# Farama-Foundation/Gymnasium-Robotics

Measured on AMD Instinct MI355X. Metric: env-steps/s (whole node), higher is better.
Workload: dtype f32

## Files before the change

gymnasium_robotics_amd/_native.py:

```python
import ctypes
import os

_HERE = os.path.dirname(os.path.abspath(__file__))
LIB_PATH = os.environ.get("GRX_HIP_LIB") or os.path.join(_HERE, "_lib", "libgrx_hip.so")
_lib = None


class OverflowLaneStruct(ctypes.Structure):
    _fields_ = [(n, ctypes.c_void_p) for n in ("skip", "entry_count", "entry_list", "list", "count", "next_flags", "next_count", "next_list", "ttl")] + [
        (n, ctypes.c_int) for n in ("soft_maxefc", "soft_jpool", "soft_maxcon", "ttl_init", "grid", "entry_cap", "next_cap")] + [
        (n, ctypes.c_void_p) for n in ("ready", "progress", "poll_list")] + [(n, ctypes.c_int) for n in ("ready_cap", "progress_total", "poll_grid", "pad_")]


class FetchBuffersStruct(ctypes.Structure):
    _fields_ = [(n, ctypes.c_void_p) for n in (
        "qpos", "qvel", "qacc_ws", "mocap", "aux", "goal", "action", "obs", "achieved", "reward", "success", "status", "mask", "order", "cost", "packed", "hullcache", "handoff")] + [
        ("handoff_stride", ctypes.c_int), ("handoff_large", ctypes.c_int), ("split_state", ctypes.c_void_p), ("split_parts", ctypes.c_int), ("sites_every_substep", ctypes.c_int), ("lane", OverflowLaneStruct)]


class FetchResetArgsStruct(ctypes.Structure):
    _fields_ = [(n, ctypes.c_void_p) for n in ("idx", "samples", "init_qpos", "init_qvel", "init_mocap")] + [("obj_qadr", ctypes.c_int), ("keep_outcome", ctypes.c_int), ("final_packed", ctypes.c_void_p)]


class PointTaskStruct(ctypes.Structure):
    _fields_ = [("n_substeps", ctypes.c_int), ("sparse_reward", ctypes.c_int), ("continuing_task", ctypes.c_int), ("agent", ctypes.c_int),
                ("goal_radius", ctypes.c_double), ("vel_clip", ctypes.c_float)]
# ... 227 lines not shown
```

gymnasium_robotics_amd/core.py:

```python
import numpy as np

from .spaces import Dict


class GoalVecEnv:

    metadata = {"render_modes": []}

    def __new__(cls, *args, **kwargs):
        obj = super().__new__(cls)
        obj._ezpickle_args, obj._ezpickle_kwargs = args, kwargs
        return obj

    def __getstate__(self):
        return {"_ezpickle_args": self._ezpickle_args, "_ezpickle_kwargs": self._ezpickle_kwargs}

    def __setstate__(self, d):
        out = type(self)(*d["_ezpickle_args"], **d["_ezpickle_kwargs"])
        self.__dict__.update(out.__dict__)
        out.__dict__.pop("_h", None)
        out.__dict__.pop("_h_big", None)
        if getattr(self, "lane", None) is not None and hasattr(self, "_lane_make_bufs"):
            self.lane._make_bufs = self._lane_make_bufs()

# ... 273 lines not shown
        import torch

        self.head = torch.zeros((n + 3) // 4 + 2, dtype=torch.int32, device=device)
        self.flags = self.head.view(torch.uint8)[:n]
        self.counts = self.head[-2:]
        self.next_list, self.entry_list = torch.zeros(n, dtype=torch.int32, device=device), torch.zeros(n, dtype=torch.int32, device=device)
        base = self.counts.data_ptr()
        self.next_count_ptr, self.entry_count_ptr = base, base + 4


ENTRY_CAP = 256


class OverflowLane:

    def __init__(self, n, device, model, make_bufs, ttl=LANE_TTL, mode="lane", lane_first=False, margin=LANE_MARGIN, poll_grid=LANE_POLL_GRID, handoff=False):
        import os
        self.mode = os.environ.get("GRX_LANE_MODE", mode)
        self.handoff = bool(handoff)
        self.entry_cap = max(ENTRY_CAP, n // 16) if self.handoff else ENTRY_CAP
        self.lane_first = bool(int(os.environ.get("GRX_LANE_FIRST", int(lane_first))))
        self.spacer = int(os.environ.get("GRX_LANE_SPACER", 0))

        import torch

        from . import _native
        from .mjcf.compiler import DIMS

        self.n, self.device = n, device
        self.cur, self.nxt, self.scratch = _LaneBuf(n, device), _LaneBuf(n, device), _LaneBuf(n, device)
        self.ttl = torch.zeros(n, dtype=torch.int8, device=device)
        dims = model.tables["dims"]
        req = lambda k, default: int(dims[DIMS.index(k + "_req")]) or default
        cap = (req("maxefc", 144), req("jpool", 2032), min(req("maxcon", 32), 32))
        margin, ttl = float(os.environ.get("GRX_LANE_MARGIN", margin)), int(os.environ.get("GRX_LANE_TTL", ttl))
        self.soft = tuple(int(margin * v) for v in cap) + (int(ttl),)
        self._make_bufs = make_bufs
        self.side = torch.cuda.Stream(device=device, priority=int(os.environ.get("GRX_LANE_PRIO", "-1")))
        self._Lane = _native.OverflowLaneStruct
        self._pin = [dict(buf=torch.zeros(2, dtype=torch.int32, pin_memory=True), event=None, age=0) for _ in range(4)]
        self._pin_next, self._seen, self._age = 0, 0, 0
        self.cap_cur = 64
        self.poll_grid = int(os.environ.get("GRX_LANE_POLL", poll_grid)) if self.mode == "lane" else 0
        self._poll = torch.zeros(self.poll_grid + 1, dtype=torch.int32, device=device) if self.poll_grid > 0 else None
        self._fast_grid = (n + 7) & ~7
# ... 97 lines not shown
            pass
        elif slot["event"] is None or slot["event"].query():
            done = torch.cuda.Event()
            done.record(main)
            self.side.wait_event(done)
            with torch.cuda.stream(self.side):
                slot["buf"].copy_(nxt.counts, non_blocking=True)
                slot["event"] = torch.cuda.Event()
                slot["event"].record(self.side)
            self._age += 1
            slot["age"] = self._age
        self.cur, self.nxt, self.cap_cur = nxt, cur, next_cap

    def rerun_only(self, mask, fast_bufs, launch_fast, launch_large):
        sc = self.scratch
        sc.head.zero_()
        fast_bufs.lane = self._fast(None, sc, 0, join=False)
        launch_fast(fast_bufs)
        fast_bufs.lane = self._Lane()
        b = self._make_bufs(mask)
        b.lane = self._large(sc.entry_list, sc.entry_count_ptr, sc, ENTRY_CAP, 0)
        launch_large(b)

    def get_state(self):
        cur = self.cur
        return dict(head=cur.head.clone(), next_list=cur.next_list.clone(), entry_list=cur.entry_list.clone(), ttl=self.ttl.clone(), cap_cur=int(self.cap_cur), seen=int(self._seen))

    def set_state(self, st):
        import torch

        cur = self.cur
        cur.head.copy_(st["head"]); cur.next_list.copy_(st["next_list"]); cur.entry_list.copy_(st["entry_list"]); self.ttl.copy_(st["ttl"])
        self.cap_cur, self._seen = int(st["cap_cur"]), int(st["seen"])
        for slot in self._pin:
            if slot["event"] is not None:
                slot["event"].synchronize()
# ... 11 lines not shown
```

gymnasium_robotics_amd/csrc/grx_engine.h:

```cpp
#pragma once
#include <math.h>
#include <stdint.h>

#if defined(GRX_EMU)
#define GRX_ON_DEVICE 0
#else
#define GRX_ON_DEVICE 1
#endif
#if GRX_ON_DEVICE && defined(GRX_PROFILE)
#define GRX_DEVICE_PROFILE 1
#else
#define GRX_DEVICE_PROFILE 0
#endif
#if defined(GRX_HULL_HINTS)
#define GRX_DEVICE_HULL_HINTS GRX_ON_DEVICE
#define GRX_TWIN_HULL_HINTS (!GRX_ON_DEVICE)
#else
#define GRX_DEVICE_HULL_HINTS 0
#define GRX_TWIN_HULL_HINTS 0
#endif
#if defined(GRX_EMU) && defined(GRX_EMU_TRACE)
#define GRX_TWIN_TRACE 1
#else
#define GRX_TWIN_TRACE 0
// ... 121 lines not shown
#define GRX_CELL_MAX 64
GRX_HD int grx_hull_cell(float x, float y, float z) {
  const float ax = fabsf(x), ay = fabsf(y), az = fabsf(z);
  int face; float ma, u, v;
  if (ax >= ay && ax >= az) { face = x < 0.0f ? 1 : 0; ma = ax; u = y; v = z; }
  else if (ay >= az) { face = y < 0.0f ? 3 : 2; ma = ay; u = x; v = z; }
  else { face = z < 0.0f ? 5 : 4; ma = az; u = x; v = y; }
  const float s = (0.5f * GRX_CELL_G) / fmaxf(ma, 1e-30f);
  int iu = (int)floorf(u * s + 0.5f * GRX_CELL_G), iv = (int)floorf(v * s + 0.5f * GRX_CELL_G);
  iu = iu < 0 ? 0 : (iu > GRX_CELL_G - 1 ? GRX_CELL_G - 1 : iu); iv = iv < 0 ? 0 : (iv > GRX_CELL_G - 1 ? GRX_CELL_G - 1 : iv);
  return (face * GRX_CELL_G + iu) * GRX_CELL_G + iv;
}
#define GRX_HULLCACHE_WORDS 90

struct GrxLane { const unsigned char* skip; int* entry_count; int* entry_list; const int* list; const int* count; unsigned char* next_flags; int* next_count; int* next_list; signed char* ttl; int soft_maxefc, soft_jpool, soft_maxcon, ttl_init, grid, entry_cap, next_cap;
                 int* ready; int* progress; const int* poll_list; int ready_cap, progress_total, poll_grid, pad_; };

struct GrxCtx {
  float *qpos, *qvel, *qacc_ws, *mocap_pos, *mocap_quat, *ctrl;
  float *ploc, *qloc, *janchor, *jaxis;
  float *xpos, *xquat, *xmat, *cinert, *crb, *cvel, *cacc, *cfrc;
  float *gxpos, *gxmat, *sxpos, *sxmat;
  float *cdof, *cdof_dot;
  float *M, *A;
  float *qfrc_bias, *qfrc_passive, *qfrc_actuator, *qfrc_smooth, *qacc_smooth, *qfrc_constraint, *qacc, *Ma, *grad, *search,
      *Mv, *tmpv;
  float *con_dist, *con_pos, *con_frame;
  int *con_pair, *con_efc, *con_nr, *con_b1, *con_b2, *con_span, *con_ioff;
  float *Jp, *efc_pos, *efc_D, *efc_aref, *efc_jar, *efc_jv, *efc_force, *efc_floss;
  int *efc_kind, *efc_id, *efc_quad, *efc_row;
  float *rk_q0, *rk_v0, *rk_Fv, *rk_Fa;
// ... 480 lines not shown
```

gymnasium_robotics_amd/csrc/grx_env.hip:

```cpp
#include <hip/hip_runtime.h>

#include <sys/random.h>

#include <cstdio>
#include <cstdlib>
#include <cstring>
#include <map>
#include <string>
#include <vector>

#include "grx_capi.h"
#include "grx_env.h"
#include "grx_replay.h"
#include "grx_episodes.h"
#include "grx_norm.h"
#include "grx_copy.h"

namespace {

constexpr int kEntryCap = 256;
constexpr int kSplitParts = 4;
constexpr int kSplitWide = 12288;
constexpr double kLaneMargin = 0.8;
constexpr int kLaneTtl = 4;
// ... 194 lines not shown
  grx_model *h = nullptr, *hbig = nullptr;
  int nq = 0, nv = 0, nmocap = 0, nu = 0, obs_dim = 0, pdim = 0, obj_qadr = -1;
  double g0[3] = {0, 0, 0}, toff[3] = {0, 0, 0}, height_offset = 0, dt = 0;
  int soft[4] = {0, 0, 0, 0};
  std::vector<void*> allocs;
  float *qpos, *qvel, *qacc_ws, *mocap, *aux, *goal, *action, *obs, *achieved, *reward, *packed, *final_packed, *final_rows, *hullcache, *cost_ema = nullptr;
  unsigned char *success, *mask;
  int *status, *cost = nullptr, *order = nullptr;
  float* split_rows = nullptr;
  int* split_state = nullptr;
  uint64_t *rng, *rng_rows;
  float *init_qpos, *init_qvel, *init_mocap;
  int *idx_main, *idx_ahead;
  float *samp_main, *samp_ahead;
  int* lane_head;
  int *lane_next_list, *lane_entry_list;
  signed char* lane_ttl;
  size_t lane_head_bytes = 0;
  float *a_qpos, *a_qvel, *a_qacc_ws, *a_mocap, *a_aux, *a_goal, *a_obs, *a_achieved, *a_reward;
  unsigned char* a_success;
  int* a_status;
  grx_fetch_buffers bufs{}, bufs_masked{}, lane_plain{}, lane_masked{}, ahead_bufs{};
  bool balance = false, ahead = false;
  bool fused_tail = true;
  int slots_per_xcd = 0, split = 1;
  hipStream_t side = nullptr;
  hipEvent_t ev_before = nullptr, ev_ahead = nullptr;
  void* pin[kPinSlots] = {};
  hipEvent_t pin_ev[kPinSlots] = {};
  bool pin_live[kPinSlots] = {};
// ... 58 lines not shown
  explicit DeviceGuard(int dev) { if (hipGetDevice(&prev) != hipSuccess) prev = -1; if (prev != dev) (void)hipSetDevice(dev); }
  ~DeviceGuard() { int cur; if (prev >= 0 && hipGetDevice(&cur) == hipSuccess && cur != prev) (void)hipSetDevice(prev); }
};

grx_fetch_buffers make_bufs(grx_env* e, float* qpos, float* qvel, float* qacc, float* mocap, float* aux, float* goal, float* obs, float* ach, float* rew, unsigned char* succ,
                            int* status, const unsigned char* mask, const int* order, int* cost, float* packed, float* hullcache) {
  grx_fetch_buffers b;
  std::memset(&b, 0, sizeof b);
  b.qpos = qpos; b.qvel = qvel; b.qacc_ws = qacc; b.mocap = mocap; b.aux = aux; b.goal = goal; b.action = e->action; b.obs = obs; b.achieved = ach;
  b.reward = rew; b.success = succ; b.status = status; b.mask = mask; b.order = order; b.cost = cost; b.packed = packed; b.hullcache = hullcache;
  return b;
}

int launch_step(grx_env* e, bool masked, bool order_now, hipStream_t s) {
  grx_fetch_buffers& fb = masked ? e->bufs_masked : e->bufs;
  ENV_HIP(hipMemsetAsync(e->lane_head, 0, e->lane_head_bytes, s));
  int* counts = e->lane_head + (e->lane_head_bytes / 4 - 2);
  std::memset(&fb.lane, 0, sizeof fb.lane);
  fb.lane.entry_count = counts + 1; fb.lane.entry_list = e->lane_entry_list; fb.lane.entry_cap = kEntryCap;
  const int rc = grx_fetch_step(e->h, &e->d.task, &fb, e->n, s);
  std::memset(&fb.lane, 0, sizeof fb.lane);
  if (rc != 0) return fail(GRX_ENV_EHIP, std::string("grx_fetch_step: ") + grx_last_error());
  grx_fetch_buffers& b = masked ? e->lane_masked : e->lane_plain;
  std::memset(&b.lane, 0, sizeof b.lane);
  b.lane.grid = kEntryCap; b.lane.list = e->lane_entry_list; b.lane.count = counts + 1;
  b.lane.next_flags = (unsigned char*)e->lane_head; b.lane.next_count = counts; b.lane.next_list = e->lane_next_list; b.lane.ttl = e->lane_ttl; b.lane.next_cap = 0;
  b.lane.soft_maxefc = e->soft[0]; b.lane.soft_jpool = e->soft[1]; b.lane.soft_maxcon = e->soft[2]; b.lane.ttl_init = e->soft[3];
  ENV_GRX(grx_fetch_step(e->hbig, &e->d.task, &b, e->n, s));
  if (e->balance && order_now) ENV_GRX(grx_order_by_cost_slots(e->cost, e->cost_ema, kBalanceAlpha, e->n, e->slots_per_xcd, e->order, s));
  return 0;
}

int sample_resets(grx_env* e, const int* idx_dev, int k, float* samples, hipStream_t s) {
  const double* c = e->d.consts;
  ENV_GRX(grx_fetch_sample_resets_device(e->rng, idx_dev, k, (int)c[0], (int)c[2], c[7], c[8], e->toff, e->g0, e->height_offset, samples, s));
  return 0;
}

int reset_inline(grx_env* e, const int* idx_dev, int k, const float* samples, bool keep_outcome, hipStream_t s) {
  grx_fetch_reset_args a;
  std::memset(&a, 0, sizeof a);
  a.idx = idx_dev; a.samples = samples; a.init_qpos = e->init_qpos; a.init_qvel = e->init_qvel; a.init_mocap = e->init_mocap; a.obj_qadr = e->obj_qadr;
  a.keep_outcome = keep_outcome ? 1 : 0; a.final_packed = keep_outcome ? e->final_packed : nullptr;
// ... 45 lines not shown
}

int alloc_all(grx_env* e) {
  const int n = e->n;
  ENV_TRY(e->zalloc(&e->qpos, (size_t)n * e->nq)); ENV_TRY(e->zalloc(&e->qvel, (size_t)n * e->nv)); ENV_TRY(e->zalloc(&e->qacc_ws, (size_t)n * e->nv));
  ENV_TRY(e->zalloc(&e->mocap, (size_t)n * 7 * e->nmocap)); ENV_TRY(e->zalloc(&e->aux, (size_t)n * 8)); ENV_TRY(e->zalloc(&e->goal, (size_t)n * 3));
  ENV_TRY(e->zalloc(&e->action, (size_t)n * 4)); ENV_TRY(e->zalloc(&e->obs, (size_t)n * e->obs_dim)); ENV_TRY(e->zalloc(&e->achieved, (size_t)n * 3));
  ENV_TRY(e->zalloc(&e->reward, n)); ENV_TRY(e->zalloc(&e->success, n)); ENV_TRY(e->zalloc(&e->status, n)); ENV_TRY(e->zalloc(&e->mask, n));
  ENV_HIP(hipMemset(e->mask, 1, n));
  ENV_TRY(e->zalloc(&e->packed, (size_t)n * e->pdim)); ENV_TRY(e->zalloc(&e->final_packed, (size_t)n * e->pdim)); ENV_TRY(e->zalloc(&e->final_rows, (size_t)n * e->pdim));
  ENV_TRY(e->zalloc(&e->hullcache, (size_t)n * kHullWords));
  ENV_TRY(e->zalloc(&e->rng, (size_t)n * 4)); ENV_TRY(e->zalloc(&e->rng_rows, (size_t)n * 4));
  ENV_TRY(e->zalloc(&e->init_qpos, e->nq)); ENV_TRY(e->zalloc(&e->init_qvel, e->nv)); ENV_TRY(e->zalloc(&e->init_mocap, 7 * e->nmocap));
  ENV_TRY(e->zalloc(&e->idx_main, n)); ENV_TRY(e->zalloc(&e->idx_ahead, n)); ENV_TRY(e->zalloc(&e->samp_main, (size_t)n * 5)); ENV_TRY(e->zalloc(&e->samp_ahead, (size_t)n * 5));
  e->lane_head_bytes = (size_t)((n + 3) / 4 + 2) * 4;
  ENV_TRY(e->zalloc(&e->lane_head, e->lane_head_bytes / 4)); ENV_TRY(e->zalloc(&e->lane_next_list, n)); ENV_TRY(e->zalloc(&e->lane_entry_list, n)); ENV_TRY(e->zalloc(&e->lane_ttl, n));
  e->balance = n % 8 == 0 && n >= 1024 && n <= 65536 * 8;
  { const char* v = std::getenv("GRX_FETCH_FUSED_TAIL"); e->fused_tail = !(v && v[0] == '0' && v[1] == 0); }
  if (e->balance) {
    ENV_TRY(e->zalloc(&e->cost, n)); ENV_TRY(e->zalloc(&e->cost_ema, n)); ENV_TRY(e->zalloc(&e->order, n));
    const int lds = grx_model_lds_bytes(e->h);
    const int granules = (lds + 1279) / 1280;
    const int per_cu = granules > 0 ? (160 * 1024) / (granules * 1280) : 8;
    e->slots_per_xcd = 32 * (per_cu < 8 ? per_cu : 8);
    std::vector<int> ord(n);
    const int per = n / 8;
    for (int j = 0; j < n; ++j) ord[j] = (j % 8) * per + j / 8;
    ENV_HIP(hipMemcpy(e->order, ord.data(), (size_t)n * 4, hipMemcpyHostToDevice));
  }
  e->bufs = make_bufs(e, e->qpos, e->qvel, e->qacc_ws, e->mocap, e->aux, e->goal, e->obs, e->achieved, e->reward, e->success, e->status, nullptr, e->order, e->cost, e->packed, e->hullcache);
  e->bufs_masked = e->bufs;
// ... 438 lines not shown
```

gymnasium_robotics_amd/csrc/grx_kernels.hip:

```cpp
#if !defined(GRX_TU_FETCH) && !defined(GRX_TU_HAND) && !defined(GRX_TU_POINT) && !defined(GRX_TU_ADROIT) && !defined(GRX_TU_KITCHEN) && !defined(GRX_TU_SIM) && !defined(GRX_TU_API)
#define GRX_TU_FETCH 1
#define GRX_TU_HAND 1
#define GRX_TU_POINT 1
#define GRX_TU_ADROIT 1
#define GRX_TU_KITCHEN 1
#define GRX_TU_SIM 1
#define GRX_TU_API 1
#endif
#if GRX_TU_FETCH && !defined(GRX_NO_HULL_HINTS)
#define GRX_HULL_HINTS 1
#endif
#include <hip/hip_runtime.h>

#include <cmath>
#include <cstdio>
#include <cstring>
#include <string>

#include "../../include/grx_capi.h"
#include "grx_fetch_task.h"
#include "grx_point_task.h"
#include "grx_hand_task.h"
#include "grx_adroit_task.h"
#include "grx_kitchen_task.h"
// ... 213 lines not shown
}
template <class S>
__global__ void __launch_bounds__(64, GRX_FETCH_WAVES(S))
grx_fetch_step_kernel(int mslot, GrxFetchTask t, GrxFetchBuffers b, int n_worlds, int words) {
  extern __shared__ float lds[];
  const int lane_ = threadIdx.x;
  const int parts = b.split_parts > 1 ? b.split_parts : 1;
  const unsigned G = gridDim.x / (unsigned)parts, part = blockIdx.x / G, slot = blockIdx.x - part * G;
  grx_fetch_step_world<S, false>(mslot, t, b, grx_slot_world(b.order, slot, G), n_worlds, words, lds, lane_, (int)part, parts);
  grx_lane_progress(b.lane);
}
template <class S>
__global__ void __launch_bounds__(64, 2)
grx_fetch_lane_kernel(int mslot, GrxFetchTask t, GrxFetchBuffers b, int n_worlds, int words) {
  extern __shared__ float lds[];
  const int e = blockIdx.x, nstand = (int)gridDim.x - b.lane.poll_grid;
  if (e >= nstand) {
    const int ent = grx_lane_poll(b.lane, e - nstand);
    if (ent < 0) return;
    if ((ent >> 30) & 1) { if (threadIdx.x == 0) atomicExch(b.lane.ready + (e - nstand), 1); return; }
    grx_fetch_step_world<S, true>(mslot, t, b, ent & 0x3FFFFFFF, n_worlds, words, lds, (int)threadIdx.x);
    return;
  }
  if (e >= *b.lane.count || grx_lane_taken(b.lane, e)) return;
  grx_fetch_step_world<S, true>(mslot, t, b, b.lane.list[e] & 0x3FFFFFFF, n_worlds, words, lds, (int)threadIdx.x);
}

template <class S>
__global__ void __launch_bounds__(64, GRX_FETCH_WAVES(S))
grx_fetch_forward_kernel(int mslot, GrxFetchTask t, GrxFetchBuffers b, int n_worlds, int words, int nstep) {
// ... 328 lines not shown
template <class S>
__global__ void __launch_bounds__(64, 2)
grx_adroit_step_kernel(int mslot, GrxAdroitTask t, GrxAdroitBuffers b, int n_worlds, int words, int forward_only) {
  extern __shared__ float lds[];
  const int lane_ = threadIdx.x;
  const int parts = (b.split_parts > 1 && !b.compact && !forward_only) ? b.split_parts : 1;
  const unsigned G = gridDim.x / (unsigned)parts, part = blockIdx.x / G, slot = blockIdx.x - part * G;
  const int w = b.compact ? ((int)blockIdx.x < b.n_compact ? (int)b.compact[blockIdx.x] : n_worlds) : grx_slot_world(b.order, slot, G);
  grx_adroit_step_world<S>(mslot, t, b, w, n_worlds, words, forward_only, lds, lane_, false, (int)part, parts);
  grx_lane_progress(b.lane);
}
template <class S>
__global__ void __launch_bounds__(64, 2)
grx_adroit_lane_kernel(int mslot, GrxAdroitTask t, GrxAdroitBuffers b, int n_worlds, int words) {
  extern __shared__ float lds[];
  const int e = blockIdx.x, nstand = (int)gridDim.x - b.lane.poll_grid;
  if (e >= nstand) { const int w = grx_lane_poll(b.lane, e - nstand); if (w >= 0) grx_adroit_step_world<S>(mslot, t, b, w, n_worlds, words, 0, lds, (int)threadIdx.x, true); return; }
  if (e >= *b.lane.count || grx_lane_taken(b.lane, e)) return;
  grx_adroit_step_world<S>(mslot, t, b, b.lane.list[e], n_worlds, words, 0, lds, (int)threadIdx.x, true);
}

#ifndef GRX_KITCHEN_CAP
#define GRX_KITCHEN_CAP 128, 1280, 0, 24
#endif
typedef GrxShape<30, 29, 9, 25, 24, 124, 0, 0, 6, 0, GRX_KITCHEN_CAP, 1, 3> GrxShapeKitchen;
typedef GrxShape<30, 29, 9, 25, 24, 124, 0, 0, 6, 0, 400, 8160, 0, 64, 1, 3> GrxShapeKitchenLane;
template <class S>
__device__ __forceinline__ void grx_kitchen_step_world(int mslot, const GrxKitchenTask& t, const GrxKitchenBuffers& b, const int w, int n_worlds, int words, int forward_only, float* lds, const int lane_, const bool in_lane,
                                                       const int part = 0, const int parts = 1) {
  if (w >= n_worlds) return;
// ... 922 lines not shown
  int fut = t + 1 + (int)(u1 * (float)(t_now - t));
  if (fut > t_now) fut = t_now;
  *t_out = t; *w_out = w;
  *tg_out = (u2 >= (float)k_future / ((float)k_future + 1.0f)) ? -1 : fut;
  return lo < t_now;
}
extern "C" __global__ void __launch_bounds__(256)
grx_her_sample_kernel(const int* __restrict__ start, const int* __restrict__ prev_start, const int* __restrict__ term_t, int N, int t_now, int T, int k_future,
                      unsigned long long seed, unsigned long long call, long long B, int* __restrict__ t_idx, int* __restrict__ w_idx, int* __restrict__ t_goal) {
  for (long long b = (long long)blockIdx.x * blockDim.x + threadIdx.x; b < B; b += (long long)gridDim.x * blockDim.x) {
    int t, w, tg;
    (void)grx_her_draw(start, prev_start, term_t, N, t_now, T, k_future, seed, call, b, &t, &w, &tg);
    t_idx[b] = t; w_idx[b] = w; t_goal[b] = tg;
  }
}
#define GRX_HER_CHUNK 32
extern "C" __global__ void __launch_bounds__(256)
grx_her_draw_relabel_kernel(GrxHerArgs a, const int* __restrict__ start, const int* __restrict__ prev_start, int t_now, int k_future, unsigned long long seed,
                            unsigned long long call, long long B, int* __restrict__ valid) {
  __shared__ int s_t[GRX_HER_CHUNK], s_w[GRX_HER_CHUNK], s_g[GRX_HER_CHUNK], s_ok[GRX_HER_CHUNK];
  const int OW = 2 * a.obs_dim + 3 * a.goal_dim + a.act_dim + 2, x = threadIdx.x;
  for (long long b0 = (long long)blockIdx.x * GRX_HER_CHUNK; b0 < B; b0 += (long long)gridDim.x * GRX_HER_CHUNK) {
    const int rows = B - b0 < GRX_HER_CHUNK ? (int)(B - b0) : GRX_HER_CHUNK;
    if (x < rows) {
      int t, w, tg;
      const bool found = grx_her_draw(start, prev_start, a.term_t, a.N, t_now, a.T, k_future, seed, call, b0 + x, &t, &w, &tg);
      s_t[x] = t; s_w[x] = w; s_g[x] = tg; s_ok[x] = (found || !valid) ? 1 : 0;
      if (valid && b0 + x == 0) *valid = found ? (int)B : 0;
    }
    __syncthreads();
    float* __restrict__ out = a.out + b0 * OW;
    for (int i = x; i < rows * OW; i += 256) {
      const int r = i / OW;
      out[i] = s_ok[r] ? grx_her_word_at(a, s_t[r], s_w[r], s_g[r], i - r * OW) : 0.0f;
// ... 18 lines not shown
                              int* t_idx, int* w_idx, int* t_goal, void* stream) {
  return grx_her_sample_final(episode_start, nullptr, nullptr, n_worlds, t_now, T, k_future, seed, call, batch, t_idx, w_idx, t_goal, stream);
}
static int grx_her_draw_relabel_impl(const char* who, const grx_her_args* args, const int* episode_start, const int* prev_start, int t_now, int k_future, uint64_t seed,
                                     uint64_t call, int64_t batch, int* valid, void* stream) {
  GrxHerArgs a; memcpy(&a, args, sizeof(a));
  if (!a.rows || !a.acts || !a.out) return fail(std::string(who) + ": null buffer");
  if ((a.term_rows == nullptr) != (a.term_t == nullptr) || (prev_start == nullptr) != (a.term_t == nullptr))
    return fail(std::string(who) + ": term_rows, term_t and prev_start go together");
  if (a.T <= 0 || a.N <= 0 || a.obs_dim <= 0 || a.goal_dim <= 0 || a.goal_dim > 16 || a.act_dim <= 0 || a.W < a.obs_dim + 2 * a.goal_dim)
    return fail(std::string(who) + ": dimensions out of range (goal_dim <= 16, W >= obs_dim + 2 goal_dim)");
  if (a.kind < 0 || a.kind > 3 || (a.kind == 0 && a.goal_dim != 3) || (a.kind == 2 && a.goal_dim != 2) || (a.kind == 3 && a.goal_dim != 7))
    return fail(std::string(who) + ": reward kind does not fit goal_dim");
  if (t_now < 0 || k_future < 0 || batch <= 0 || batch > (1ll << 30)) return fail(std::string(who) + ": t_now, k_future >= 0 and 1 <= batch <= 2^30");
  a.t_idx = a.w_idx = a.t_goal = nullptr;
  long long blocks = (batch + GRX_HER_CHUNK - 1) / GRX_HER_CHUNK;
  if (blocks > 4096) blocks = 4096;
  hipLaunchKernelGGL(grx_her_draw_relabel_kernel, dim3((unsigned)blocks), dim3(256), 0, (hipStream_t)stream, a, episode_start, prev_start, t_now, k_future,
                     (unsigned long long)seed, (unsigned long long)call, (long long)batch, valid);
  HIP_OK(hipGetLastError());
  return 0;
}
extern "C" int grx_her_draw_relabel(const grx_her_args* args, const int* episode_start, const int* prev_start, int t_now, int k_future, uint64_t seed, uint64_t call,
                                    int64_t batch, int* valid, void* stream) {
  if (!args || !episode_start) return fail("grx_her_draw_relabel: null argument");
  if (!valid && t_now <= 0) return fail("grx_her_draw_relabel: without valid the caller vouches for a world with a transition (t_now > 0)");
  return grx_her_draw_relabel_impl("grx_her_draw_relabel", args, episode_start, prev_start, t_now, k_future, seed, call, batch, valid, stream);
}
extern "C" int grx_her_sample_relabel(const grx_her_args* args, const int* episode_start, const int* prev_start, int t_now, int k_future, uint64_t seed, uint64_t call,
                                      int64_t batch, int* scratch, int* valid, void* stream) {
  if (!args || !episode_start || !scratch || !valid) return fail("grx_her_sample_relabel: null argument");
  return grx_her_draw_relabel_impl("grx_her_sample_relabel", args, episode_start, prev_start, t_now, k_future, seed, call, batch, valid, stream);
}
// ... 846 lines not shown
```

gymnasium_robotics_amd/csrc/grx_step_frame.h:

```cpp
#pragma once
#include "grx_engine.h"

static __device__ __forceinline__ int grx_slot_world(const int* order, unsigned slot, unsigned G) { return order ? order[slot] : (int)((slot & 7u) * (G >> 3) + (slot >> 3)); }
static __device__ __forceinline__ int grx_slot_world_late(const int* order, int parts) {
  unsigned bx = blockIdx.x; asm volatile("" : "+s"(bx));
  const unsigned G = parts > 1 ? gridDim.x / (unsigned)parts : gridDim.x, slot = parts > 1 ? bx % G : bx;
  return grx_slot_world(order, slot, G);
}

__device__ __forceinline__ void grx_lane_setup(const GrxLane& L, GrxCtx& c, int w, bool stepping) {
  c.bail = (stepping && L.entry_count != nullptr) ? 1 : 0;
  if (c.bail) { c.lane_entry_count = L.entry_count; c.lane_entry_list = L.entry_list; c.lane_entry_cap = L.entry_cap; c.lane_world = w; c.lane_ready = L.ready; c.lane_ready_cap = L.ready_cap; }
  if (stepping && (L.list != nullptr || L.entry_count != nullptr)) { c.soft_maxefc = L.soft_maxefc; c.soft_jpool = L.soft_jpool; c.soft_maxcon = L.soft_maxcon; }
}
__device__ __forceinline__ bool grx_lane_overflowed(const GrxCtx& c) { return c.bail == 2; }
__device__ __forceinline__ void grx_lane_append(const GrxLane& L, int w) {
  const int idx = atomicAdd(L.next_count, 1);
  if (idx < L.next_cap) { L.next_list[idx] = w; L.next_flags[w] = 1; }
}
__device__ __forceinline__ void grx_lane_join(const GrxLane& L, const GrxCtx& c, int w, int lane_) {
  if (L.entry_count == nullptr || L.next_list == nullptr || lane_ != 0 || !(c.cnt[2] & GRX_ST_SOFT)) return;
  L.ttl[w] = (signed char)L.ttl_init;
  grx_lane_append(L, w);
}
// ... 14 lines not shown
__device__ __forceinline__ int grx_lane_poll(const GrxLane& L, int p) {
  if (!L.ready || p >= L.ready_cap) return -1;
  int w = -1;
  if (threadIdx.x == 0) {
    for (int it = 0; it < 40000; it++) {
      int r = __hip_atomic_load(L.ready + p, __ATOMIC_RELAXED, __HIP_MEMORY_SCOPE_AGENT);
      if (r == 0 && __hip_atomic_load(L.progress, __ATOMIC_RELAXED, __HIP_MEMORY_SCOPE_AGENT) >= L.progress_total)
        r = __hip_atomic_load(L.ready + p, __ATOMIC_RELAXED, __HIP_MEMORY_SCOPE_AGENT);
      else if (r == 0) { __builtin_amdgcn_s_sleep(127); __builtin_amdgcn_s_sleep(127); continue; }
      if (r == 1 && atomicCAS(L.ready + p, 1, 2) == 1) { __threadfence(); w = ((volatile const int*)L.poll_list)[p]; }
      break;
    }
  }
  return __builtin_amdgcn_readfirstlane(w);
}
template <class STEP>
__device__ __forceinline__ void grx_lane_walk(const GrxLane& L, STEP step) {
  const int e = blockIdx.x, nstand = (int)gridDim.x - L.poll_grid;
  if (e >= nstand) { const int w = grx_lane_poll(L, e - nstand); if (w >= 0) step(w); return; }
  if (e >= *L.count || grx_lane_taken(L, e)) return;
  step(L.list[e]);
}

template <class P, class O>
__device__ __forceinline__ void grx_state_load(GrxCtx& c, P qpos, O oq, P qvel, O ov, P qacc, O oa, int nq, int nv, int lane_) {
  for (int i = lane_; i < nq; i += 64) c.qpos[i] = qpos[oq + i];
  for (int i = lane_; i < nv; i += 64) { c.qvel[i] = qvel[ov + i]; c.qacc_ws[i] = qacc[oa + i]; }
}
template <class P, class O>
__device__ __forceinline__ void grx_state_store(const GrxCtx& c, P qpos, O oq, P qvel, O ov, P qacc, O oa, int nq, int nv, int lane_) {
  for (int i = lane_; i < nq; i += 64) qpos[oq + i] = c.qpos[i];
  for (int i = lane_; i < nv; i += 64) { qvel[ov + i] = c.qvel[i]; qacc[oa + i] = c.qacc_ws[i]; }
// ... 51 lines not shown
```

gymnasium_robotics_amd/envs/fetch.py:

```python
import ctypes
import os
from typing import Optional

import numpy as np
import torch

from .. import _native
from ..core import create_rerun_model, GoalVecEnv, OverflowLane, np_random
from ..mjcf import CompiledModel, compile_mjcf, load_model
from ..spaces import Box, Dict, batch_space
from .fetch_spec import DISTANCE_THRESHOLD, FETCH_TASKS, MAX_EPISODE_STEPS, N_SUBSTEPS, make_fetch_task, parse_env_id

_MODELS_DIR = os.path.join(os.path.dirname(os.path.abspath(__file__)), "..", "models")


FETCH_CAPACITY = {"maxcon": 28, "maxefc": 144, "jpool": 2032, "split_spans": False}
FETCH_FAST_CAPACITY = {"maxcon": 24, "maxefc": 96, "jpool": 1024}
FETCH_SPLIT_PARTS = 4
FETCH_SPLIT_WIDE = 12288
HANDOFF_TASKS = ("FetchPickAndPlace",)


def load_fetch_model(task: str, assets_root: Optional[str] = None) -> CompiledModel:
    xml = FETCH_TASKS[task]["xml"]
# ... 17 lines not shown
    if cfg["has_object"]:
        oxy = g0[:2]
        while np.linalg.norm(oxy - g0[:2]) < 0.1:
            oxy = g0[:2] + rng.uniform(-cfg["obj_range"], cfg["obj_range"], size=2)
    goal = g0[:3] + rng.uniform(-cfg["target_range"], cfg["target_range"], size=3)
    if cfg["has_object"]:
        goal = goal + cfg["target_offset"]
        goal[2] = height_offset
        if cfg["target_in_the_air"] and rng.uniform() < 0.5:
            goal[2] += rng.uniform(0, 0.45)
    return oxy, goal


class FetchVecEnv(GoalVecEnv):

    CKPT_SKIP = GoalVecEnv.CKPT_SKIP + ("_ahead",)

    def __init__(self, env_id: str = "FetchPickAndPlace-v4", num_envs: int = 1, device: Optional[str] = None,
                 max_episode_steps: Optional[int] = MAX_EPISODE_STEPS, autoreset_mode: str = "next_step",
                 output: str = "numpy", assets_root: Optional[str] = None, model: Optional[CompiledModel] = None,
                 reward_type: Optional[str] = None, seed_offset: int = 0, balance: bool = True, overflow_rerun: bool = True):
        task, rt = parse_env_id(env_id)
        self.balance = balance
        self.env_id, self.task_name, self.reward_type = env_id, task, reward_type or rt
        self.cfg = FETCH_TASKS[task]
        self.num_envs = int(num_envs)
        self.max_episode_steps = max_episode_steps
        if autoreset_mode not in ("next_step", "same_step", "disabled"):
            raise ValueError(f"unknown autoreset_mode {autoreset_mode}")
        self.autoreset_mode, self.output = autoreset_mode, output
        self.seed_offset = int(seed_offset)
# ... 58 lines not shown
            self.lane.step(self.mask if bufs is self._bufs_masked else None, fast, large, fast_bufs=bufs, launch_lane=middle)
            if timed:
                l1.record()
                self.step_events.append((l0, l1))
        if self.balance:
            if self._defer_order:
                self._order_pending = True
            else:
                self._rebalance()

    def _alloc(self, n):
        d, f32 = self.device, torch.float32
        z = lambda *s, dtype=f32: torch.zeros(*s, dtype=dtype, device=d)
        self.qpos, self.qvel, self.qacc_ws = z(n, self.nq), z(n, self.nv), z(n, self.nv)
        self.mocap, self.aux, self.goal, self.action = z(n, 7 * self.nmocap), z(n, 8), z(n, 3), z(n, 4)
        self.obs, self.achieved, self.reward = z(n, self.obs_dim), z(n, 3), z(n)
        self.success, self.status = z(n, dtype=torch.uint8), z(n, dtype=torch.int32)
        self.mask = torch.ones(n, dtype=torch.uint8, device=d)
        self.balance = bool(self.balance) and n % 8 == 0 and 1024 <= n <= 65536 * 8
        self._reset_stage = z(n, 6)
        self._fused = os.environ.get("GRX_FETCH_FUSED_TAIL", "1") != "0"
        self._defer_order, self._order_pending = False, False
        self.step_reset_list = None
        self.packed = z(n, self.obs_dim + 8)
        self.final_packed = z(n, self.obs_dim + 8)
        self.cost = torch.zeros(n, dtype=torch.int32, device=d) if self.balance else None
        self.cost_ema = torch.zeros(n, dtype=torch.float32, device=d) if self.balance else None
        self.balance_alpha = float(os.environ.get("GRX_BALANCE_ALPHA", 0.1))
        self.order = None
        self._slots_per_xcd = 32 * min(12 if self._h_fast else 8, (160 * 1024) // (-(-self.lds_bytes // 1280) * 1280)) if (self.balance and os.environ.get("GRX_TAIL_ORDER", "1") != "0") else 0
# ... 9 lines not shown
            self.handoff = z(n, self._handoff_stride)
        self._bufs = self._make_bufs(*common, None, self.order, self.cost, self.packed, self.hullcache, self.handoff)
        self._bufs_masked = self._make_bufs(*common, self.mask, self.order, self.cost, self.packed, self.hullcache, self.handoff)
        self._bufs.handoff_stride = self._bufs_masked.handoff_stride = self._handoff_stride
        sites_every = int(os.environ.get("GRX_FETCH_SITES_EVERY_SUBSTEP", "0") != "0")
        self._bufs.sites_every_substep = self._bufs_masked.sites_every_substep = sites_every
        self._split = max(1, int(os.environ.get("GRX_FETCH_SPLIT", str((FETCH_SPLIT_PARTS if n <= FETCH_SPLIT_WIDE else 2) if n > 2048 else 1)))) if self.handoff is None and n >= 64 else 1
        if self._split > 1:
            stride = -(-(2 + self.model.dim("nu") + 7 * self.nmocap + self.nq + 2 * self.nv) // 16) * 16
            self._split_rows, self._split_state = z(n, stride), z(n, 2, dtype=torch.int32)
            for b in (self._bufs, self._bufs_masked):
                b.handoff, b.handoff_stride, b.split_state, b.split_parts = self._split_rows.data_ptr(), stride, self._split_state.data_ptr(), self._split
        self.lane = None
        if self._h_big is not None:
            packed, hullcache, handoff, stride, mk = self.packed, self.hullcache, self.handoff, self._handoff_stride, FetchVecEnv._make_bufs

            def lane_bufs(m):
                b = mk(*common, m, None, None, packed, hullcache, handoff)
                b.handoff_stride, b.sites_every_substep = stride, sites_every
                return b

            if handoff is not None:
                self.lane = OverflowLane(n, d, self._fast_model, lane_bufs, mode="lane", handoff=True, poll_grid=int(os.environ.get("GRX_FETCH_POLL", max(64, n // 32))),
                                         ttl=int(os.environ.get("GRX_FETCH_TTL", 4)), margin=0.9)
            else:
                self.lane = OverflowLane(n, d, self.model, lane_bufs, mode="entry")
        self._ahead = None
        if n > 1 and os.environ.get("GRX_FETCH_AHEAD_RESET", "1") != "0":
            sq, sv, sa, sm, sx, sg, so, sh = z(n, self.nq), z(n, self.nv), z(n, self.nv), z(n, 7 * self.nmocap), z(n, 8), z(n, 3), z(n, self.obs_dim), z(n, 3)
            sr, ss, st = z(n), z(n, dtype=torch.uint8), z(n, dtype=torch.int32)
            self._ahead = dict(qpos=sq, qvel=sv, qacc_ws=sa, mocap=sm, aux=sx, goal=sg, obs=so, achieved=sh, reward=sr, success=ss, status=st)
            self._ahead_bufs = self._make_bufs(sq, sv, sa, sm, sx, sg, self.action, so, sh, sr, ss, st, None, None, None, None, None)
            self._ahead_stream = torch.cuda.Stream(device=d)
# ... 124 lines not shown
        if len(idx) == 0:
            return None
        staged = self._stage_reset(idx)
        self._launch_reset(staged, idx)
        return staged[1].long()

    def reset(self, *, seed=None, options=None):
        if seed is not None:
            seeds = [seed + self.seed_offset + i for i in range(self.num_envs)] if np.isscalar(seed) else list(seed)
            self._seed_worlds(seeds)
        with torch.cuda.device(self.device):
            self._reset_worlds(np.arange(self.num_envs))
        self._has_reset, self.step_reset_list = True, None
        return self._obs_dict(), {}

    def step(self, actions):
        if not self._has_reset:
            raise RuntimeError("Cannot call env.step() before calling env.reset()")
        if isinstance(actions, torch.Tensor):
            if tuple(actions.shape) != (self.num_envs, 4):
                raise ValueError("Action dimension mismatch")
            self.action.copy_(actions.to(torch.float32), non_blocking=True)
        else:
            a = np.asarray(actions, dtype=np.float32)
            if a.shape != (self.num_envs, 4):
                raise ValueError("Action dimension mismatch")
            self.action.copy_(torch.from_numpy(a), non_blocking=True)
        with torch.cuda.device(self.device):
            pending = np.nonzero(self._needs_reset)[0] if self.autoreset_mode == "next_step" else np.zeros(0, np.int64)
            ahead, will, before = None, np.zeros(0, np.int64), None
            if self._ahead is not None and self.autoreset_mode == "same_step" and self.max_episode_steps is not None:
                will = np.nonzero(self._elapsed + 1 >= self.max_episode_steps)[0]
                if len(will) and self._ahead_late:
                    before = torch.cuda.Event()
                    before.record(torch.cuda.current_stream(self.device))
                elif len(will):
                    ahead = (will, self._launch_reset_ahead(will))
            self.step_reset_list = None
            if self._order_pending:
                self._post_step()
            self._defer_order = self._fused and self.autoreset_mode == "same_step" and not len(pending)
# ... 106 lines not shown
```

include/grx_capi.h:

```cpp
#ifndef GRX_CAPI_H
#define GRX_CAPI_H

#include <stdint.h>

#ifdef __cplusplus
extern "C" {
#endif

typedef struct grx_model grx_model;

typedef struct grx_overflow_lane {
  const unsigned char* skip;
  int* entry_count; int* entry_list;
  const int* list; const int* count;
  unsigned char* next_flags; int* next_count; int* next_list;
  signed char* ttl;
  int soft_maxefc, soft_jpool, soft_maxcon, ttl_init;
  int grid;
  int entry_cap, next_cap;
  int* ready; int* progress; const int* poll_list;
  int ready_cap, progress_total, poll_grid, pad_;
} grx_overflow_lane;

typedef struct grx_fetch_task {
  int has_object, block_gripper, n_substeps, sparse_reward;
  int grip_body;
  float grip_relpos[3], grip_relquat[4];
  int site_grip, site_obj;
  int jq_rf, jq_lf, jd_rf, jd_lf;
  int obs_dim, goal_dim;
  float dt;
  double distance_threshold;
} grx_fetch_task;

enum grx_status_bits {
  GRX_STATUS_BADNUM = 1,
// ... 334 lines not shown
```

Before: 1.498 million.

## Fold lane-head clearing into lane kernel, zero-copy actions, regroup HER relabel

The per-step hipMemsetAsync of the lane head buffer is replaced by double-buffered heads: the lane kernel zeroes the other head buffer for the next step, which removes one launch per step. The Fetch env now reads contiguous float32 device action tensors in place instead of copying them into its own buffer. The HER relabel kernel gets a new default layout that maps 16 threads to each sample, and the old chunked kernel stays available through an environment variable. The risks are aliasing a caller-owned action tensor that may change before the kernel runs, and ordering hazards on the swapped head buffers.

Measured after the change: 1.511 million, median of 6. No clear change (+0.8%).

```diff
diff --git a/gymnasium_robotics_amd/_native.py b/gymnasium_robotics_amd/_native.py
--- a/gymnasium_robotics_amd/_native.py
+++ b/gymnasium_robotics_amd/_native.py
@@ -9,7 +9,8 @@
 class OverflowLaneStruct(ctypes.Structure):
     _fields_ = [(n, ctypes.c_void_p) for n in ("skip", "entry_count", "entry_list", "list", "count", "next_flags", "next_count", "next_list", "ttl")] + [
         (n, ctypes.c_int) for n in ("soft_maxefc", "soft_jpool", "soft_maxcon", "ttl_init", "grid", "entry_cap", "next_cap")] + [
-        (n, ctypes.c_void_p) for n in ("ready", "progress", "poll_list")] + [(n, ctypes.c_int) for n in ("ready_cap", "progress_total", "poll_grid", "pad_")]
+        (n, ctypes.c_void_p) for n in ("ready", "progress", "poll_list")] + [(n, ctypes.c_int) for n in ("ready_cap", "progress_total", "poll_grid", "pad_")] + [
+        ("clear_head", ctypes.c_void_p), ("clear_words", ctypes.c_int), ("pad2_", ctypes.c_int)]
 
 
 class FetchBuffersStruct(ctypes.Structure):
diff --git a/gymnasium_robotics_amd/core.py b/gymnasium_robotics_amd/core.py
--- a/gymnasium_robotics_amd/core.py
+++ b/gymnasium_robotics_amd/core.py
@@ -311,7 +311,7 @@
 
 class OverflowLane:
 
-    def __init__(self, n, device, model, make_bufs, ttl=LANE_TTL, mode="lane", lane_first=False, margin=LANE_MARGIN, poll_grid=LANE_POLL_GRID, handoff=False):
+    def __init__(self, n, device, model, make_bufs, ttl=LANE_TTL, mode="lane", lane_first=False, margin=LANE_MARGIN, poll_grid=LANE_POLL_GRID, handoff=False, head_fill=False):
         import os
         self.mode = os.environ.get("GRX_LANE_MODE", mode)
         self.handoff = bool(handoff)
@@ -326,6 +326,8 @@
 
         self.n, self.device = n, device
         self.cur, self.nxt, self.scratch = _LaneBuf(n, device), _LaneBuf(n, device), _LaneBuf(n, device)
+        self._scratch_other = _LaneBuf(n, device)
+        self.head_fill = bool(int(os.environ.get("GRX_LANE_HEAD_FILL", int(head_fill))))
         self.ttl = torch.zeros(n, dtype=torch.int8, device=device)
         dims = model.tables["dims"]
         req = lambda k, default: int(dims[DIMS.index(k + "_req")]) or default
@@ -453,12 +455,19 @@
 
     def rerun_only(self, mask, fast_bufs, launch_fast, launch_large):
         sc = self.scratch
-        sc.head.zero_()
+        if self.head_fill:
+            sc.head.zero_()
+        else:
+            self.scratch, self._scratch_other = self._scratch_other, sc
+            sc = self.scratch
         fast_bufs.lane = self._fast(None, sc, 0, join=False)
         launch_fast(fast_bufs)
         fast_bufs.lane = self._Lane()
         b = self._make_bufs(mask)
         b.lane = self._large(sc.entry_list, sc.entry_count_ptr, sc, ENTRY_CAP, 0)
+        if not self.head_fill:
+            other = self._scratch_other
+            b.lane.clear_head, b.lane.clear_words = other.head.data_ptr(), other.head.numel()
         launch_large(b)
 
     def get_state(self):
diff --git a/gymnasium_robotics_amd/csrc/grx_engine.h b/gymnasium_robotics_amd/csrc/grx_engine.h
--- a/gymnasium_robotics_amd/csrc/grx_engine.h
+++ b/gymnasium_robotics_amd/csrc/grx_engine.h
@@ -159,7 +159,8 @@
 #define GRX_HULLCACHE_WORDS 90
 
 struct GrxLane { const unsigned char* skip; int* entry_count; int* entry_list; const int* list; const int* count; unsigned char* next_flags; int* next_count; int* next_list; signed char* ttl; int soft_maxefc, soft_jpool, soft_maxcon, ttl_init, grid, entry_cap, next_cap;
-                 int* ready; int* progress; const int* poll_list; int ready_cap, progress_total, poll_grid, pad_; };
+                 int* ready; int* progress; const int* poll_list; int ready_cap, progress_total, poll_grid, pad_;
+                 int* clear_head; int clear_words, pad2_; };
 
 struct GrxCtx {
   float *qpos, *qvel, *qacc_ws, *mocap_pos, *mocap_quat, *ctrl;
diff --git a/gymnasium_robotics_amd/csrc/grx_env.hip b/gymnasium_robotics_amd/csrc/grx_env.hip
--- a/gymnasium_robotics_amd/csrc/grx_env.hip
+++ b/gymnasium_robotics_amd/csrc/grx_env.hip
@@ -7,6 +7,7 @@
 #include <cstring>
 #include <map>
 #include <string>
+#include <utility>
 #include <vector>
 
 #include "grx_capi.h"
@@ -232,6 +233,7 @@
   int *idx_main, *idx_ahead;
   float *samp_main, *samp_ahead;
   int* lane_head;
+  int* lane_head_other;
   int *lane_next_list, *lane_entry_list;
   signed char* lane_ttl;
   size_t lane_head_bytes = 0;
@@ -320,8 +322,8 @@
 
 int launch_step(grx_env* e, bool masked, bool order_now, hipStream_t s) {
   grx_fetch_buffers& fb = masked ? e->bufs_masked : e->bufs;
-  ENV_HIP(hipMemsetAsync(e->lane_head, 0, e->lane_head_bytes, s));
-  int* counts = e->lane_head + (e->lane_head_bytes / 4 - 2);
+  int* const head = e->lane_head;
+  int* counts = head + (e->lane_head_bytes / 4 - 2);
   std::memset(&fb.lane, 0, sizeof fb.lane);
   fb.lane.entry_count = counts + 1; fb.lane.entry_list = e->lane_entry_list; fb.lane.entry_cap = kEntryCap;
   const int rc = grx_fetch_step(e->h, &e->d.task, &fb, e->n, s);
@@ -330,9 +332,11 @@
   grx_fetch_buffers& b = masked ? e->lane_masked : e->lane_plain;
   std::memset(&b.lane, 0, sizeof b.lane);
   b.lane.grid = kEntryCap; b.lane.list = e->lane_entry_list; b.lane.count = counts + 1;
-  b.lane.next_flags = (unsigned char*)e->lane_head; b.lane.next_count = counts; b.lane.next_list = e->lane_next_list; b.lane.ttl = e->lane_ttl; b.lane.next_cap = 0;
+  b.lane.clear_head = e->lane_head_other; b.lane.clear_words = (int)(e->lane_head_bytes / 4);
+  b.lane.next_flags = (unsigned char*)head; b.lane.next_count = counts; b.lane.next_list = e->lane_next_list; b.lane.ttl = e->lane_ttl; b.lane.next_cap = 0;
   b.lane.soft_maxefc = e->soft[0]; b.lane.soft_jpool = e->soft[1]; b.lane.soft_maxcon = e->soft[2]; b.lane.ttl_init = e->soft[3];
   ENV_GRX(grx_fetch_step(e->hbig, &e->d.task, &b, e->n, s));
+  std::swap(e->lane_head, e->lane_head_other);
   if (e->balance && order_now) ENV_GRX(grx_order_by_cost_slots(e->cost, e->cost_ema, kBalanceAlpha, e->n, e->slots_per_xcd, e->order, s));
   return 0;
 }
@@ -408,7 +412,7 @@
   ENV_TRY(e->zalloc(&e->init_qpos, e->nq)); ENV_TRY(e->zalloc(&e->init_qvel, e->nv)); ENV_TRY(e->zalloc(&e->init_mocap, 7 * e->nmocap));
   ENV_TRY(e->zalloc(&e->idx_main, n)); ENV_TRY(e->zalloc(&e->idx_ahead, n)); ENV_TRY(e->zalloc(&e->samp_main, (size_t)n * 5)); ENV_TRY(e->zalloc(&e->samp_ahead, (size_t)n * 5));
   e->lane_head_bytes = (size_t)((n + 3) / 4 + 2) * 4;
-  ENV_TRY(e->zalloc(&e->lane_head, e->lane_head_bytes / 4)); ENV_TRY(e->zalloc(&e->lane_next_list, n)); ENV_TRY(e->zalloc(&e->lane_entry_list, n)); ENV_TRY(e->zalloc(&e->lane_ttl, n));
+  ENV_TRY(e->zalloc(&e->lane_head, e->lane_head_bytes / 4)); ENV_TRY(e->zalloc(&e->lane_head_other, e->lane_head_bytes / 4)); ENV_TRY(e->zalloc(&e->lane_next_list, n)); ENV_TRY(e->zalloc(&e->lane_entry_list, n)); ENV_TRY(e->zalloc(&e->lane_ttl, n));
   e->balance = n % 8 == 0 && n >= 1024 && n <= 65536 * 8;
   { const char* v = std::getenv("GRX_FETCH_FUSED_TAIL"); e->fused_tail = !(v && v[0] == '0' && v[1] == 0); }
   if (e->balance) {
diff --git a/gymnasium_robotics_amd/csrc/grx_kernels.hip b/gymnasium_robotics_amd/csrc/grx_kernels.hip
--- a/gymnasium_robotics_amd/csrc/grx_kernels.hip
+++ b/gymnasium_robotics_amd/csrc/grx_kernels.hip
@@ -251,6 +251,7 @@
 __global__ void __launch_bounds__(64, 2)
 grx_fetch_lane_kernel(int mslot, GrxFetchTask t, GrxFetchBuffers b, int n_worlds, int words) {
   extern __shared__ float lds[];
+  grx_lane_clear(b.lane);
   const int e = blockIdx.x, nstand = (int)gridDim.x - b.lane.poll_grid;
   if (e >= nstand) {
     const int ent = grx_lane_poll(b.lane, e - nstand);
@@ -609,6 +610,7 @@
 __global__ void __launch_bounds__(64, 2)
 grx_adroit_lane_kernel(int mslot, GrxAdroitTask t, GrxAdroitBuffers b, int n_worlds, int words) {
   extern __shared__ float lds[];
+  grx_lane_clear(b.lane);
   const int e = blockIdx.x, nstand = (int)gridDim.x - b.lane.poll_grid;
   if (e >= nstand) { const int w = grx_lane_poll(b.lane, e - nstand); if (w >= 0) grx_adroit_step_world<S>(mslot, t, b, w, n_worlds, words, 0, lds, (int)threadIdx.x, true); return; }
   if (e >= *b.lane.count || grx_lane_taken(b.lane, e)) return;
@@ -1561,10 +1563,24 @@
     t_idx[b] = t; w_idx[b] = w; t_goal[b] = tg;
   }
 }
-#define GRX_HER_CHUNK 32
+#define GRX_HER_GROUP 16
 extern "C" __global__ void __launch_bounds__(256)
 grx_her_draw_relabel_kernel(GrxHerArgs a, const int* __restrict__ start, const int* __restrict__ prev_start, int t_now, int k_future, unsigned long long seed,
                             unsigned long long call, long long B, int* __restrict__ valid) {
+  const int OW = 2 * a.obs_dim + 3 * a.goal_dim + a.act_dim + 2, lane_ = threadIdx.x & (GRX_HER_GROUP - 1);
+  for (long long b = (long long)blockIdx.x * (256 / GRX_HER_GROUP) + threadIdx.x / GRX_HER_GROUP; b < B; b += (long long)gridDim.x * (256 / GRX_HER_GROUP)) {
+    int t, w, tg;
+    bool ok = grx_her_draw(start, prev_start, a.term_t, a.N, t_now, a.T, k_future, seed, call, b, &t, &w, &tg);
+    if (valid && b == 0 && lane_ == 0) *valid = ok ? (int)B : 0;
+    if (!valid) ok = true;
+    float* __restrict__ out = a.out + b * OW;
+    for (int e = lane_; e < OW; e += GRX_HER_GROUP) out[e] = ok ? grx_her_word_at(a, t, w, tg, e) : 0.0f;
+  }
+}
+#define GRX_HER_CHUNK 32
+extern "C" __global__ void __launch_bounds__(256)
+grx_her_draw_relabel_chunk_kernel(GrxHerArgs a, const int* __restrict__ start, const int* __restrict__ prev_start, int t_now, int k_future, unsigned long long seed,
+                                  unsigned long long call, long long B, int* __restrict__ valid) {
   __shared__ int s_t[GRX_HER_CHUNK], s_w[GRX_HER_CHUNK], s_g[GRX_HER_CHUNK], s_ok[GRX_HER_CHUNK];
   const int OW = 2 * a.obs_dim + 3 * a.goal_dim + a.act_dim + 2, x = threadIdx.x;
   for (long long b0 = (long long)blockIdx.x * GRX_HER_CHUNK; b0 < B; b0 += (long long)gridDim.x * GRX_HER_CHUNK) {
@@ -1613,9 +1629,12 @@
     return fail(std::string(who) + ": reward kind does not fit goal_dim");
   if (t_now < 0 || k_future < 0 || batch <= 0 || batch > (1ll << 30)) return fail(std::string(who) + ": t_now, k_future >= 0 and 1 <= batch <= 2^30");
   a.t_idx = a.w_idx = a.t_goal = nullptr;
-  long long blocks = (batch + GRX_HER_CHUNK - 1) / GRX_HER_CHUNK;
+  static const bool chunk = getenv("GRX_HER_LAYOUT") && !strcmp(getenv("GRX_HER_LAYOUT"), "chunk");
+  const long long per = chunk ? GRX_HER_CHUNK : 256 / GRX_HER_GROUP;
+  long long blocks = (batch + per - 1) / per;
   if (blocks > 4096) blocks = 4096;
-  hipLaunchKernelGGL(grx_her_draw_relabel_kernel, dim3((unsigned)blocks), dim3(256), 0, (hipStream_t)stream, a, episode_start, prev_start, t_now, k_future,
+  auto kern = chunk ? grx_her_draw_relabel_chunk_kernel : grx_her_draw_relabel_kernel;
+  hipLaunchKernelGGL(kern, dim3((unsigned)blocks), dim3(256), 0, (hipStream_t)stream, a, episode_start, prev_start, t_now, k_future,
                      (unsigned long long)seed, (unsigned long long)call, (long long)batch, valid);
   HIP_OK(hipGetLastError());
   return 0;
diff --git a/gymnasium_robotics_amd/csrc/grx_step_frame.h b/gymnasium_robotics_amd/csrc/grx_step_frame.h
--- a/gymnasium_robotics_amd/csrc/grx_step_frame.h
+++ b/gymnasium_robotics_amd/csrc/grx_step_frame.h
@@ -52,8 +52,13 @@
   }
   return __builtin_amdgcn_readfirstlane(w);
 }
+__device__ __forceinline__ void grx_lane_clear(const GrxLane& L) {
+  if (L.clear_head == nullptr) return;
+  for (int i = (int)(blockIdx.x * blockDim.x + threadIdx.x); i < L.clear_words; i += (int)(gridDim.x * blockDim.x)) L.clear_head[i] = 0;
+}
 template <class STEP>
 __device__ __forceinline__ void grx_lane_walk(const GrxLane& L, STEP step) {
+  grx_lane_clear(L);
   const int e = blockIdx.x, nstand = (int)gridDim.x - L.poll_grid;
   if (e >= nstand) { const int w = grx_lane_poll(L, e - nstand); if (w >= 0) step(w); return; }
   if (e >= *L.count || grx_lane_taken(L, e)) return;
diff --git a/gymnasium_robotics_amd/envs/fetch.py b/gymnasium_robotics_amd/envs/fetch.py
--- a/gymnasium_robotics_amd/envs/fetch.py
+++ b/gymnasium_robotics_amd/envs/fetch.py
@@ -55,7 +55,7 @@
 
 class FetchVecEnv(GoalVecEnv):
 
-    CKPT_SKIP = GoalVecEnv.CKPT_SKIP + ("_ahead",)
+    CKPT_SKIP = GoalVecEnv.CKPT_SKIP + ("_ahead", "_action_src")
 
     def __init__(self, env_id: str = "FetchPickAndPlace-v4", num_envs: int = 1, device: Optional[str] = None,
                  max_episode_steps: Optional[int] = MAX_EPISODE_STEPS, autoreset_mode: str = "next_step",
@@ -144,6 +144,7 @@
         z = lambda *s, dtype=f32: torch.zeros(*s, dtype=dtype, device=d)
         self.qpos, self.qvel, self.qacc_ws = z(n, self.nq), z(n, self.nv), z(n, self.nv)
         self.mocap, self.aux, self.goal, self.action = z(n, 7 * self.nmocap), z(n, 8), z(n, 3), z(n, 4)
+        self._action_src, self._action_ptr, self._action_copy = self.action, [self.action.data_ptr()], os.environ.get("GRX_FETCH_ACTION_COPY", "0") == "1"
         self.obs, self.achieved, self.reward = z(n, self.obs_dim), z(n, 3), z(n)
         self.success, self.status = z(n, dtype=torch.uint8), z(n, dtype=torch.int32)
         self.mask = torch.ones(n, dtype=torch.uint8, device=d)
@@ -183,9 +184,11 @@
         self.lane = None
         if self._h_big is not None:
             packed, hullcache, handoff, stride, mk = self.packed, self.hullcache, self.handoff, self._handoff_stride, FetchVecEnv._make_bufs
+            act_ptr = self._action_ptr
 
             def lane_bufs(m):
                 b = mk(*common, m, None, None, packed, hullcache, handoff)
+                b.action = act_ptr[0]
                 b.handoff_stride, b.sites_every_substep = stride, sites_every
                 return b
 
@@ -340,17 +343,29 @@
         self._has_reset, self.step_reset_list = True, None
         return self._obs_dict(), {}
 
+    def _read_actions_from(self, t):
+        ptr = t.data_ptr()
+        if self._action_src is not t or self._action_ptr[0] != ptr:
+            self._action_src = t
+            self._action_ptr[0] = ptr
+            self._bufs.action = self._bufs_masked.action = ptr
+
     def step(self, actions):
         if not self._has_reset:
             raise RuntimeError("Cannot call env.step() before calling env.reset()")
         if isinstance(actions, torch.Tensor):
             if tuple(actions.shape) != (self.num_envs, 4):
                 raise ValueError("Action dimension mismatch")
-            self.action.copy_(actions.to(torch.float32), non_blocking=True)
+            if not self._action_copy and actions.dtype == torch.float32 and actions.device == self.action.device and actions.is_contiguous():
+                self._read_actions_from(actions)
+            else:
+                self._read_actions_from(self.action)
+                self.action.copy_(actions.to(torch.float32), non_blocking=True)
         else:
             a = np.asarray(actions, dtype=np.float32)
             if a.shape != (self.num_envs, 4):
                 raise ValueError("Action dimension mismatch")
+            self._read_actions_from(self.action)
             self.action.copy_(torch.from_numpy(a), non_blocking=True)
         with torch.cuda.device(self.device):
             pending = np.nonzero(self._needs_reset)[0] if self.autoreset_mode == "next_step" else np.zeros(0, np.int64)
diff --git a/include/grx_capi.h b/include/grx_capi.h
--- a/include/grx_capi.h
+++ b/include/grx_capi.h
@@ -20,6 +20,7 @@
   int entry_cap, next_cap;
   int* ready; int* progress; const int* poll_list;
   int ready_cap, progress_total, poll_grid, pad_;
+  int* clear_head; int clear_words, pad2_;
 } grx_overflow_lane;
 
 typedef struct grx_fetch_task {
```
